# pierluigiferrari/ssd_keras

Hardware: AMD Instinct MI355X
Metric: images/sec SSD300 fwd+decode @batch32 (higher is better)
Workload: dtype f32 (decode, threshold, TF-style f32 NMS, top-k); bf16 conv backbone; 1 GPU; SSD300 VGG-16 inference (mode='inference': forward + DecodeDetections), 21 classes, batch 32 per GPU, conf 0.01 / NMS 0.45 / top-200, random-init weights, synthetic 300x300x3 uint8-range images; per_gpu_batch=32, global_batch=32, conv_dtype=bf16, parallelism=replicas x1, launch=hip_graph (forward + DecodeDetections captured once, replayed per step), decode_stream=same stream; DecodeDetections reads the head outputs directly (no y_pred in HBM)

## Files before the change

### ssd_keras_amd/csrc/ssdhip_convh.hip

```cpp
#include <hip/hip_runtime.h>
#include <stdint.h>
#include <stdlib.h>

#include <type_traits>

#include "ssdhip.h"
#include "ssdhip_math.h"

namespace ssdhip {

#ifdef SSDHIP_PROFILE
__device__ unsigned long long g_profh[16];
#define CH_PROF_DECL long long _pt = clock64(); long long _pa[4] = {0, 0, 0, 0}; int _pn = 0;
#define CH_PROF_MARK(i) { const long long _t = clock64(); _pa[i] += _t - _pt; _pt = _t; }
#define CH_PROF_TILE ++_pn;
#define CH_PROF_FLUSH(base) if ((threadIdx.x & 63) == 0) { for (int _i = 0; _i < 4; ++_i) atomicAdd(&g_profh[(base) + _i], (unsigned long long)_pa[_i]); atomicAdd(&g_profh[(base) + 4], (unsigned long long)_pn); }
#else
#define CH_PROF_DECL
#define CH_PROF_MARK(i)
#define CH_PROF_TILE
#define CH_PROF_FLUSH(base)
#endif

typedef unsigned short bf16_t;
// ... 41 lines not shown
__device__ __forceinline__ u32 ch_pkmax_i16(u32 a, u32 b) {
    return __builtin_bit_cast(u32, __builtin_elementwise_max(__builtin_bit_cast(ch_s16x2, a), __builtin_bit_cast(ch_s16x2, b)));
}

__device__ __forceinline__ void ch_bload(u32 voff, i32x4 rsrc, u32 lds_dst, u32 soff) {
    u32 keep;
    lds_dst = (u32)__builtin_amdgcn_readfirstlane((int)lds_dst);
    soff = (u32)__builtin_amdgcn_readfirstlane((int)soff);
    asm volatile("s_mov_b32 %0, m0\n\ts_mov_b32 m0, %3\n\ts_nop 0\n\tbuffer_load_dwordx4 %1, %2, %4 offen lds\n\ts_mov_b32 m0, %0"
                 : "=&s"(keep) : "v"(voff), "s"(rsrc), "s"(lds_dst), "s"(soff) : "memory");
}
__device__ __forceinline__ i32x4 ch_rsrc(const void* base, int num_records) {
    const unsigned long long a = (unsigned long long)(uintptr_t)base;
    i32x4 r;
    r.x = (int)(u32)a;
    r.y = (int)((u32)(a >> 32) & 0xffffu);
    r.z = num_records;
    r.w = 0x00020000;
    return r;
}
__device__ __forceinline__ u32 ch_keep2(u32 m) {
    const ch_s16x2 h = __builtin_bit_cast(ch_s16x2, m);
    const ch_s16x2 a = h & (short)0x7fff;
    const ch_s16x2 k = (h > (short)0) | (a > (short)0x7f80);
    return __builtin_bit_cast(u32, k);
}
typedef _Float16 ch_f16x8 __attribute__((ext_vector_type(8)));
__device__ __forceinline__ u32 ch_split2(float a, float b, u32& lo_out) {
    const _Float16 ha = (_Float16)a, hb = (_Float16)b;
    const _Float16 la = (_Float16)(a - (float)ha), lb = (_Float16)(b - (float)hb);
    lo_out = (u32)__builtin_bit_cast(unsigned short, la) | ((u32)__builtin_bit_cast(unsigned short, lb) << 16);
    return (u32)__builtin_bit_cast(unsigned short, ha) | ((u32)__builtin_bit_cast(unsigned short, hb) << 16);
}

template <int NW, int SPW, int MODE, int CSH, bool POOL, bool SMALL, bool X3 = false, int NWV = 8, bool STK = false, bool MSK = false,
          bool KEEP = false>
__device__ __forceinline__ void convh_body(const ConvHParams& p, unsigned char* lds, const int first_id) {
    constexpr bool G2 = CSH != 0;
    static_assert(!KEEP || (POOL && !X3 && NWV == 8 && !(MODE & (16384 | 1024))), "KEEP: the staged pooled bf16 epilogue, plain waits");
    static_assert(!MSK || (!POOL && !X3 && NWV == 8 && !(MODE & 16384)), "masked outputs: the staged bf16 epilogue without pooling");
    static_assert(!STK || (POOL && !((MODE & 16384) != 0 && !X3)), "stacked-batch tiles: the staged pooled epilogues");
    static_assert(NWV == 8 || (NWV == 4 && !X3), "8 waves, or 4 (bf16 forms only)");
    constexpr int NPI = 16 / NWV;
    constexpr int WPK = 8 / NWV;
    constexpr int TC = G2 ? (1 << CSH) : 1, TR = G2 ? (CH_BN >> CSH) : 1, SC2 = TC + 2;
    static_assert(!POOL || G2, "the pooled epilogue needs 2-D tiles");
    static_assert(!G2 || (TR + 2) * (TC + 2) <= 64 * SPW, "the 2-D slab must fit the slab buffer");
    constexpr bool LZ = (MODE & 8192) != 0 && NW == 4;
    constexpr int D = LZ ? NW - 1 : NW;
    constexpr int SLAB0 = NW * CH_WST, SLB = SPW * 8192;
    constexpr unsigned OOB = 0x80000000u;
    constexpr bool PERSIST = (MODE & 128) != 0;
    static_assert(SPW + D <= 10, "slice cs+1's slab must have landed two steps before tap 8 of slice cs reads it");
    static_assert(SLB >= 32768, "the epilogue stages half a tile (8 waves x 32 positions x 128 B) in the idle slab buffer");

    auto tile_of = [&](const int id, int& q0, int& co0) {
        const int xcd = id & 7, slot = id >> 3;
        const int qt = (slot / p.n_tiles) * 8 + xcd;
        q0 = G2 ? qt : qt * CH_BN;
        co0 = (slot % p.n_tiles) * CH_BM;
        return id < p.total_ids && qt < p.q_tiles;
    };
    int id = first_id, q0, co0;
    if (!tile_of(id, q0, co0)) {
        if constexpr (MSK) {
            if (p.bsum) {
                const int w_ = (int)threadIdx.x >> 6, l_ = (int)threadIdx.x & 63;
                const int slot_ = first_id >> 3, cz = (slot_ % p.n_tiles) * CH_BM + (w_ >> 2) * 64 + l_;
                p.bsum[(size_t)(4 * ((slot_ / p.n_tiles) * 8 + (first_id & 7)) + (w_ & 3)) * p.Cout + cz] = 0.f;
            }
        }
        return;
    }

    const int tid = threadIdx.x, lane = tid & 63;
// ... 68 lines not shown
        }
        int q = tile_q0 - (W + 2) + row0;
        int b = 0, h = 0, w = 0;
        if (q >= 0) { b = q / (H1 * W1); const int r = q - b * (H1 * W1); h = r / W1; w = r - h * W1; }
        else { w = q; }
#pragma unroll
        for (int k = 0; k < NXO; ++k) {
            const int row = row0 + XSTEP * k;
            const int j = (lane & 7) ^ ((row >> 1) & 7);
            const bool ok = w >= 0 && w < W && h < H && q < p.Q && row < SP;
            xoff[k] = ok ? (u32)(((b * H + h) * W + w) * (XC * 2) + j * 16) : OOB;
            q += XSTEP;
            w += XSTEP;
            while (w >= W1) { w -= W1; if (++h == H1) { h = 0; ++b; } }
        }
    };
    make_xoff(q0);
    auto xdst = [&](const int k) { return (u32)((XSTEP * k + 8 * wave) * 128); };
    constexpr int NWP = 2 * WPK;
    u32 woff[NWP];
#pragma unroll
    for (int i = 0; i < NWP; ++i) {
        const int row = (i * NWV + wave) * 8 + (lane >> 3);
        const int j = (lane & 7) ^ ((row >> 1) & 7);
        woff[i] = (u32)(row * (9 * Cin * 2) + j * 16);
    }

    auto issue_w_piece = [&](const int co, const int cs, const int tap, const int stage, const int i) {
        const u32 soff = (u32)(((co * 9 + tap) * Cin + cs * 64) * 2);
        ch_bload(woff[i], rw, lds0 + stage * CH_WST + (i * NWV + wave) * 1024, soff);
    };

    u32 abase[4];
    {
        const int row = wm * 64 + r31;
#pragma unroll
        for (int kk = 0; kk < 4; ++kk) abase[kk] = (u32)(row * 128 + (((2 * kk + khalf) ^ ((row >> 1) & 7)) << 4));
    }
    const int slot2 = wn * (16 * NPI) + r31;
    const int prow = G2 ? (2 * (slot2 >> CSH)) * SC2 + (slot2 & (TC - 1)) : wn * (32 * NPI) + r31;
    auto pirow = [&](const int pi) {
        return G2 ? (pi >> 1) * (2 * (32 >> CSH)) * SC2 + (pi & 1) * SC2 : pi * 32;
    };

    f32x16 acc[2][NPI];
    bf16x8 fa[2][4][2], fb[2][4][NPI];

    u32 ra[4], rb[NPI], re[NPI];
    auto read_addr = [&](const int cs, const int tap, const int stage) {
        u32 wst = (u32)(stage * CH_WST);
        u32 toff = (u32)((tap / 3) * (G2 ? SC2 : W1) + tap % 3);
        u32 sl = (u32)(SLAB0 + (cs & 1) * SLB);
        asm volatile("" : "+s"(wst), "+s"(toff), "+s"(sl));
#pragma unroll
        for (int kk = 0; kk < 4; ++kk) ra[kk] = abase[kk] + wst;
#pragma unroll
        for (int pi = 0; pi < NPI; ++pi) {
            const u32 row = (u32)(prow + pirow(pi)) + toff;
            rb[pi] = sl + (row << 7);
            re[pi] = (((row >> 1) & 7u) ^ (u32)khalf) << 4;
        }
    };
    constexpr int RPK = 2 + NPI;
    auto read_one = [&](auto setc, auto jc) {
        constexpr int S = decltype(setc)::value, j = decltype(jc)::value, kk = j / RPK, w = j % RPK;
        if constexpr (w < 2) fa[S][kk][w] = *reinterpret_cast<const bf16x8*>(lds + ra[kk] + w * 4096);
        else fb[S][kk][w - 2] = *reinterpret_cast<const bf16x8*>(lds + rb[w - 2] + (re[w - 2] ^ (u32)(kk << 5)));
    };
    auto mfma_one = [&](auto setc, auto ic) {
        constexpr int S = decltype(setc)::value, i = decltype(ic)::value, kk = i / (2 * NPI), ci = (i / NPI) & 1, pi = i % NPI;
        if constexpr (X3)
            acc[ci][pi] = __builtin_amdgcn_mfma_f32_32x32x16_f16(__builtin_bit_cast(ch_f16x8, fa[S][kk][ci]), __builtin_bit_cast(ch_f16x8, fb[S][kk][pi]),
                                                                 acc[ci][pi], 0, 0, 0);
        else
            acc[ci][pi] = __builtin_amdgcn_mfma_f32_32x32x16_bf16(fa[S][kk][ci], fb[S][kk][pi], acc[ci][pi], 0, 0, 0);
    };
    using I0 = std::integral_constant<int, 0>; using I1 = std::integral_constant<int, 1>;

#pragma unroll
    for (int k = 0; k < NXO; ++k) ch_bload(xoff[k], rx, lds0 + SLAB0 + xdst(k), 0u);
#pragma unroll
    for (int d = 0; d < D; ++d)
#pragma unroll
        for (int i = 0; i < NWP; ++i) issue_w_piece(co0, 0, d, d, i);
    asm volatile("s_waitcnt vmcnt(%0)" :: "n"(NWP * (D - 2)) : "memory");
    __builtin_amdgcn_s_barrier();
    read_addr(0, 0, 0);
#pragma unroll
    for (int kk = 0; kk < 4; ++kk) {
#pragma unroll
        for (int ci = 0; ci < 2; ++ci) fa[0][kk][ci] = *reinterpret_cast<const bf16x8*>(lds + ra[kk] + ci * 4096);
#pragma unroll
        for (int pi = 0; pi < NPI; ++pi) fb[0][kk][pi] = *reinterpret_cast<const bf16x8*>(lds + rb[pi] + (re[pi] ^ (u32)(kk << 5)));
    }

    int vbase = 0;
    bool has_next = false;
    int q0n = 0, co0n = 0;

    auto step = [&](auto grpc, auto setc, auto tapc, const int cs, const bool nomore, const bool nxt) {
        constexpr int GRP = decltype(grpc)::value, S = decltype(setc)::value, TAP = decltype(tapc)::value;
        using Sn = std::integral_constant<int, 1 - S>;
        constexpr auto issued = [](int t, bool lst) { return (lst ? (t < 9 - D ? 2 : 0) : 2 + (t < SPW ? 1 : 0)) * WPK; };
        constexpr int n_mid = (D == 3 ? 0 : (TAP > 0 ? issued(TAP - 1, false) : 2 * WPK)) + issued(TAP, false);
        constexpr int n_last = (D == 3 ? 0 : (TAP > 0 ? issued(TAP - 1, true) : 2 * WPK)) + issued(TAP, true);
        const int vs = vbase + cs;
        const bool post = cs == 0 && vbase > 0;
        const int st = NW == 3 ? (TAP + D) % 3 : ((vs + TAP + D) & 3);
        constexpr int RSH = ((MODE & 64) && GRP) ? 2 : 0, QSH = ((MODE & 8) && GRP) ? 2 : 0;
        auto addr_now = [&]() { read_addr(cs + (TAP == 8 ? 1 : 0), (TAP + 1) % 9, NW == 3 ? (TAP + 1) % 3 : ((vs + TAP + 1) & 3)); };
        auto req_w = [&](const int wi) {
            constexpr bool CARRY = TAP + D >= 9;
            if (!nomore || !CARRY) {
                const bool over = CARRY && nxt;
                issue_w_piece(over ? co0n : co0, over ? 0 : cs + (CARRY ? 1 : 0), (TAP + D) % 9, st, wi);
            }
        };
        auto req_x = [&](const int u) {
            if (!nomore)
                ch_bload(xoff[TAP * WPK + u], rx, lds0 + SLAB0 + ((cs + 1) & 1) * SLB + xdst(TAP * WPK + u),
                         nxt ? 0u : (u32)(((X3 && cs + 1 >= p.nx) ? cs + 1 - p.nx : cs + 1) * 128));
        };
        auto slot = [&](auto ic) {
            constexpr int i = decltype(ic)::value, j = i - RSH;
            __builtin_amdgcn_sched_barrier(0);
            if constexpr (!(MODE & 32)) mfma_one(setc, ic);
            __builtin_amdgcn_sched_barrier(0);
            if constexpr (i == 0) {
                addr_now();
                __builtin_amdgcn_sched_barrier(0);
            }
            if constexpr (NWV == 8) {
                if constexpr (!(MODE & 2)) {
                    if constexpr (j >= 0 && j < 4) {
                        read_one(Sn{}, std::integral_constant<int, 2 * (j < 0 ? 0 : j)>{});
                        read_one(Sn{}, std::integral_constant<int, 2 * (j < 0 ? 0 : j) + 1>{});
                    } else if constexpr (j >= 4 && j < 12) {
                        read_one(Sn{}, std::integral_constant<int, (j < 4 ? 4 : j) + 4>{});
                    }
                }
                if constexpr (!(MODE & 1)) {
                    if constexpr (i == 1 + QSH) req_w(0);
                    else if constexpr (i == 5 + QSH) req_w(1);
                    else if constexpr (i == 9 + QSH && TAP < SPW) req_x(0);
                }
            } else {
                if constexpr (!(MODE & 2) && i < 24) read_one(Sn{}, std::integral_constant<int, (i < 24 ? i : 0)>{});
                if constexpr (!(MODE & 1)) {
                    if constexpr (i == 2) req_w(0);
                    else if constexpr (i == 6) req_w(1);
                    else if constexpr (i == 10) req_w(2);
                    else if constexpr (i == 14) req_w(3);
                    else if constexpr ((i == 18 || i == 22) && TAP < SPW) req_x(i == 18 ? 0 : 1);
                }
            }
        };
        slot(std::integral_constant<int, 0>{}); slot(std::integral_constant<int, 1>{}); slot(std::integral_constant<int, 2>{});
        slot(std::integral_constant<int, 3>{}); slot(std::integral_constant<int, 4>{}); slot(std::integral_constant<int, 5>{});
        slot(std::integral_constant<int, 6>{}); slot(std::integral_constant<int, 7>{}); slot(std::integral_constant<int, 8>{});
        slot(std::integral_constant<int, 9>{}); slot(std::integral_constant<int, 10>{}); slot(std::integral_constant<int, 11>{});
        slot(std::integral_constant<int, 12>{}); slot(std::integral_constant<int, 13>{}); slot(std::integral_constant<int, 14>{});
        slot(std::integral_constant<int, 15>{});
        if constexpr (NWV == 4) {
            slot(std::integral_constant<int, 16>{}); slot(std::integral_constant<int, 17>{}); slot(std::integral_constant<int, 18>{});
            slot(std::integral_constant<int, 19>{}); slot(std::integral_constant<int, 20>{}); slot(std::integral_constant<int, 21>{});
            slot(std::integral_constant<int, 22>{}); slot(std::integral_constant<int, 23>{}); slot(std::integral_constant<int, 24>{});
            slot(std::integral_constant<int, 25>{}); slot(std::integral_constant<int, 26>{}); slot(std::integral_constant<int, 27>{});
            slot(std::integral_constant<int, 28>{}); slot(std::integral_constant<int, 29>{}); slot(std::integral_constant<int, 30>{});
            slot(std::integral_constant<int, 31>{});
        }
        __builtin_amdgcn_sched_barrier(0);
        if constexpr (!(MODE & 4)) {
            constexpr bool TOL = (MODE & 1024) != 0 && TAP < D - 2;
            if constexpr (LZ) {
                if (TOL && post) asm volatile("s_waitcnt vmcnt(%0)" :: "n"((MODE & 1) ? 0 : n_mid + NST + 1) : "memory");
                else if (!nomore) asm volatile("s_waitcnt vmcnt(%0)" :: "n"((MODE & 1) ? 0 : n_mid) : "memory");
                else asm volatile("s_waitcnt vmcnt(%0)" :: "n"((MODE & 1) ? 0 : n_last) : "memory");
            } else {
            if (TOL && post) asm volatile("s_waitcnt vmcnt(%0) lgkmcnt(0)" :: "n"((MODE & 1) ? 0 : n_mid + NST + 1) : "memory");
            else if (!nomore) asm volatile("s_waitcnt vmcnt(%0) lgkmcnt(0)" :: "n"((MODE & 1) ? 0 : n_mid) : "memory");
            else asm volatile("s_waitcnt vmcnt(%0) lgkmcnt(0)" :: "n"((MODE & 1) ? 0 : n_last) : "memory");
            }
            __builtin_amdgcn_s_barrier();
        }
    };
    auto slice = [&](auto grpc, auto parc, const int cs, const bool nomore, const bool nxt) {
        constexpr int P = decltype(parc)::value;
        using A = std::integral_constant<int, P>; using B = std::integral_constant<int, 1 - P>;
        step(grpc, A{}, std::integral_constant<int, 0>{}, cs, nomore, nxt); step(grpc, B{}, std::integral_constant<int, 1>{}, cs, nomore, nxt);
        step(grpc, A{}, std::integral_constant<int, 2>{}, cs, nomore, nxt); step(grpc, B{}, std::integral_constant<int, 3>{}, cs, nomore, nxt);
        step(grpc, A{}, std::integral_constant<int, 4>{}, cs, nomore, nxt); step(grpc, B{}, std::integral_constant<int, 5>{}, cs, nomore, nxt);
        step(grpc, A{}, std::integral_constant<int, 6>{}, cs, nomore, nxt); step(grpc, B{}, std::integral_constant<int, 7>{}, cs, nomore, nxt);
        step(grpc, A{}, std::integral_constant<int, 8>{}, cs, nomore, nxt);
    };
    auto k_loop = [&](auto grpc) {
        for (int cs = 0; cs < csteps; cs += 2) {
            const bool fin = cs + 2 >= csteps;
            slice(grpc, I0{}, cs, false, false);
            if (PERSIST && fin && has_next) make_xoff(q0n);
            slice(grpc, I1{}, cs + 1, fin && !has_next, fin && has_next);
        }
    };

    CH_PROF_DECL
    for (;;) {
        if constexpr (PERSIST) has_next = tile_of(id + (int)gridDim.x, q0n, co0n);
        u32 bias_dw;
        {
            const bf16_t* bsrc = (p.bias ? p.bias + co0 + wm * 64 : p.w) + 2 * r31;
            asm volatile("global_load_dword %0, %1, off" : "=v"(bias_dw) : "v"(bsrc) : "memory");
        }
#pragma unroll
        for (int ci = 0; ci < 2; ++ci)
#pragma unroll
            for (int pi = 0; pi < NPI; ++pi)
#pragma unroll
                for (int v = 0; v < 16; ++v) acc[ci][pi][v] = 0.f;
        if constexpr ((MODE & (8 | 64)) != 0) {
            if (wave < 4) k_loop(I0{}); else k_loop(I1{});
        } else {
            k_loop(I0{});
        }

        asm volatile("" : "+v"(bias_dw));
        CH_PROF_MARK(0)
        if constexpr ((MODE & 512) != 0) {
            asm volatile("" :: "v"(acc[0][0]), "v"(acc[0][1]), "v"(acc[1][0]), "v"(acc[1][1]));
            if constexpr (NPI == 4) asm volatile("" :: "v"(acc[0][2]), "v"(acc[0][3]), "v"(acc[1][2]), "v"(acc[1][3]));
        } else {
        unsigned char* stage = lds + SLAB0 + SLB + wave * 4096;
        float bv[2][16];
        if (!p.bias) bias_dw = 0u;
        const float rfloor = p.relu ? 0.f : -__builtin_inff();
        if constexpr (X3) {
#pragma unroll
            for (int ci = 0; ci < 2; ++ci)
#pragma unroll
                for (int g = 0; g < 4; ++g)
#pragma unroll
                    for (int e = 0; e < 4; ++e)
                        bv[ci][4 * g + e] = p.bias32 ? p.bias32[co0 + wm * 64 + ci * 32 + 8 * g + 4 * khalf + e] : 0.f;
        } else
#pragma unroll
        for (int ci = 0; ci < 2; ++ci)
#pragma unroll
            for (int g = 0; g < 4; ++g) {
                const int dw = ci * 16 + 4 * g + 2 * khalf;
                const u32 lo = (u32)__builtin_amdgcn_ds_bpermute(dw * 4, (int)bias_dw);
                const u32 hi = (u32)__builtin_amdgcn_ds_bpermute(dw * 4 + 4, (int)bias_dw);
                bv[ci][4 * g + 0] = __uint_as_float(lo << 16);
                bv[ci][4 * g + 1] = __uint_as_float(lo & 0xffff0000u);
                bv[ci][4 * g + 2] = __uint_as_float(hi << 16);
                bv[ci][4 * g + 3] = __uint_as_float(hi & 0xffff0000u);
            }
        if constexpr (!X3) {
        const u32 floor16 = p.relu ? 0u : 0x80008000u;
        auto pack4 = [&](const int ci, const int pi, const int g, u32& p0, u32& p1) {
            const float s0 = acc[ci][pi][4 * g + 0] + bv[ci][4 * g + 0], s1 = acc[ci][pi][4 * g + 1] + bv[ci][4 * g + 1];
            const float s2 = acc[ci][pi][4 * g + 2] + bv[ci][4 * g + 2], s3 = acc[ci][pi][4 * g + 3] + bv[ci][4 * g + 3];
            p0 = ch_pkmax_i16(ch_pack2(s0, s1), floor16);
            p1 = ch_pkmax_i16(ch_pack2(s2, s3), floor16);
        };
        auto store_runs = [&](const u32 (&lo)[4], const u32 (&hi)[4], const u32 off) {
#pragma unroll
            for (int pr = 0; pr < 2; ++pr) {
                const auto sl = __builtin_amdgcn_permlane32_swap(lo[2 * pr], lo[2 * pr + 1], false, false);
                const auto sh = __builtin_amdgcn_permlane32_swap(hi[2 * pr], hi[2 * pr + 1], false, false);
                store16_at(make_uint4(sl[0], sh[0], sl[1], sh[1]), off + pr * 32);
            }
        };
        if constexpr (POOL && DIRECT) {
            static_assert(NPI == 2, "eight-wave form");
            int b, h0, w0;
            tile_origin(q0, b, h0, w0);
// ... 223 lines not shown
                            q += 8;
                            w += 8;
                            if (!SMALL || W1 >= 8) {
                                const bool wr = w >= W1;
                                w -= wr ? W1 : 0;
                                h += wr ? 1 : 0;
                                const bool hr = h == H1;
                                h = hr ? 0 : h;
                                b += hr ? 1 : 0;
                            } else {
                                while (w >= W1) { w -= W1; if (++h == H1) { h = 0; ++b; } }
                            }
                        }
                }
            }
            [[maybe_unused]] ch_u32x4 mk[NPI][4];
            [[maybe_unused]] float bs[8] = {0.f, 0.f, 0.f, 0.f, 0.f, 0.f, 0.f, 0.f};
            [[maybe_unused]] float4 bold0 = make_float4(0.f, 0.f, 0.f, 0.f), bold1 = bold0;
            [[maybe_unused]] float* brow = nullptr;
            if constexpr (MSK) {
                const __amdgpu_buffer_rsrc_t rm = __builtin_amdgcn_make_buffer_rsrc(const_cast<bf16_t*>(p.mask), 0, p.y_bytes, 0x00020000);
#pragma unroll
                for (int pi = 0; pi < NPI; ++pi)
#pragma unroll
                    for (int j = 0; j < 4; ++j) mk[pi][j] = __builtin_amdgcn_raw_buffer_load_b128(rm, soff[pi][j], 0, 0);
                if (p.bsum && lane < 8) {
                    const int slot0 = first_id >> 3;
                    brow = p.bsum + (size_t)(4 * ((slot0 / p.n_tiles) * 8 + (first_id & 7)) + wn) * p.Cout + co0 + wm * 64 + lane * 8;
                    if (id != first_id) { bold0 = reinterpret_cast<const float4*>(brow)[0]; bold1 = reinterpret_cast<const float4*>(brow)[1]; }
                }
            }
#pragma unroll
            for (int pi = 0; pi < NPI; ++pi) {
#pragma unroll
                for (int ci = 0; ci < 2; ++ci)
#pragma unroll
                    for (int g = 0; g < 4; ++g) {
                        u32 p0, p1;
                        pack4(ci, pi, g, p0, p1);
                        const int chunk = ci * 4 + g;
                        *reinterpret_cast<uint2*>(stage + r31 * 128 + ((chunk ^ (r31 & 7)) << 4) + khalf * 8) = make_uint2(p0, p1);
                    }
                asm volatile("s_waitcnt lgkmcnt(0)" ::: "memory");
#pragma unroll
                for (int j = 0; j < 4; ++j) {
                    const int px = j * 8 + (lane >> 3);
                    uint4 v = *reinterpret_cast<const uint4*>(stage + px * 128 + ((c ^ (px & 7)) << 4));
                    if constexpr (MSK) {
                        v.x &= ch_keep2(mk[pi][j][0]); v.y &= ch_keep2(mk[pi][j][1]);
                        v.z &= ch_keep2(mk[pi][j][2]); v.w &= ch_keep2(mk[pi][j][3]);
                        bs[0] += __uint_as_float(v.x << 16); bs[1] += __uint_as_float(v.x & 0xffff0000u);
                        bs[2] += __uint_as_float(v.y << 16); bs[3] += __uint_as_float(v.y & 0xffff0000u);
                        bs[4] += __uint_as_float(v.z << 16); bs[5] += __uint_as_float(v.z & 0xffff0000u);
                        bs[6] += __uint_as_float(v.w << 16); bs[7] += __uint_as_float(v.w & 0xffff0000u);
                    }
                    store16_at(v, soff[pi][j]);
                }
                asm volatile("s_waitcnt lgkmcnt(0)" ::: "memory");
            }
            if constexpr (MSK) {
                if (p.bsum) {
#pragma unroll
                    for (int q = 0; q < 8; ++q) {
                        bs[q] += __shfl_xor(bs[q], 8);
                        bs[q] += __shfl_xor(bs[q], 16);
                        bs[q] += __shfl_xor(bs[q], 32);
// ... 120 lines not shown
                        w += 8;
                        if (!SMALL || W1 >= 8) {
                            const bool wr = w >= W1;
                            w -= wr ? W1 : 0;
                            h += wr ? 1 : 0;
                            const bool hr = h == H1;
                            h = hr ? 0 : h;
                            b += hr ? 1 : 0;
                        } else {
                            while (w >= W1) { w -= W1; if (++h == H1) { h = 0; ++b; } }
                        }
                    }
                }
                asm volatile("s_waitcnt lgkmcnt(0)" ::: "memory");
              }
            }
        }
        }
        CH_PROF_MARK(1)
        CH_PROF_TILE
        if (!has_next) break;
        __builtin_amdgcn_s_barrier();
        CH_PROF_MARK(2)
        id += (int)gridDim.x;
        q0 = q0n;
        co0 = co0n;
        vbase += csteps;
    }
    if (wave == 0) { CH_PROF_FLUSH(0) }
    if (wave == 4) { CH_PROF_FLUSH(8) }
}
#endif

template <int NW, int SPW, int MODE, int CSH, bool POOL, bool X3 = false, int NWV = 8, bool STK = false, bool MSK = false, bool KEEP = false>
__global__ __launch_bounds__(64 * NWV) void convh_kernel(ConvHParams p) {
#if defined(__HIP_DEVICE_COMPILE__)
    __shared__ __attribute__((aligned(1024))) unsigned char lds[ch_lds_bytes(NW, SPW)];
    convh_body<NW, SPW, MODE, CSH, POOL, SPW == 5, X3, NWV, STK, MSK, KEEP>(p, lds, (int)blockIdx.x);
#endif
}

constexpr int CH_MAX_GROUP = 8;
struct ConvHGroup {
    ConvHParams p[CH_MAX_GROUP];
    int first_id[CH_MAX_GROUP + 1];
    int n;
};

template <int MODE>
__global__ __launch_bounds__(CH_THREADS) void convh_group_kernel(ConvHGroup g) {
#if defined(__HIP_DEVICE_COMPILE__)
    __shared__ __attribute__((aligned(1024))) unsigned char lds[ch_lds_bytes(4, 6)];
    const int G = (int)gridDim.x, total = g.first_id[g.n];
    for (int round = 0;; ++round) {
        const int id = (round & 1) ? (round + 1) * G - 1 - (int)blockIdx.x : round * G + (int)blockIdx.x;
        if (round * G >= total) break;
        if (id >= total) continue;
        int k = 0;
        while (k + 1 < g.n && id >= g.first_id[k + 1]) ++k;
        convh_body<4, 6, MODE, 0, false, true>(g.p[k], lds, id - g.first_id[k]);
    }
#endif
}

constexpr bool convh_has_stk(int mode, bool x3) { return x3 ? mode == 128 : mode == 1152; }
template <int MODE, bool X3 = false>
static void convh_launch(const ConvHParams& p, int geom, int pool, int n_cu, hipStream_t stream) {
    int grid = p.total_ids;
    if ((MODE & 128) && grid > n_cu) grid = n_cu;
    if constexpr ((MODE & 4096) != 0 && !X3) {
        constexpr int M4 = MODE & ~4096;
        const dim3 g(grid), t(256);
        if (geom == 4) {
            if (pool) hipLaunchKernelGGL((convh_kernel<4, 6, M4, 4, true, false, 4>), g, t, 0, stream, p);
            else hipLaunchKernelGGL((convh_kernel<4, 6, M4, 4, false, false, 4>), g, t, 0, stream, p);
        } else if (geom == 5) {
            if (pool) hipLaunchKernelGGL((convh_kernel<4, 6, M4, 5, true, false, 4>), g, t, 0, stream, p);
            else hipLaunchKernelGGL((convh_kernel<4, 6, M4, 5, false, false, 4>), g, t, 0, stream, p);
        }
        else if (p.W <= 30) hipLaunchKernelGGL((convh_kernel<4, 5, M4, 0, false, false, 4>), g, t, 0, stream, p);
        else if (p.W <= 62) hipLaunchKernelGGL((convh_kernel<4, 6, M4, 0, false, false, 4>), g, t, 0, stream, p);
        else hipLaunchKernelGGL((convh_kernel<3, 7, M4, 0, false, false, 4>), g, t, 0, stream, p);
    } else {
    const dim3 g(grid), t(CH_THREADS);
    if constexpr ((MODE & 2048) != 0) {
        if (p.W <= 30) hipLaunchKernelGGL((convh_kernel<4, 5, MODE, 0, false, X3>), g, t, 0, stream, p);
        else if (p.W <= 62) hipLaunchKernelGGL((convh_kernel<4, 6, MODE, 0, false, X3>), g, t, 0, stream, p);
        else hipLaunchKernelGGL((convh_kernel<3, 7, MODE, 0, false, X3>), g, t, 0, stream, p);
    } else
    if (geom == 4) {
        if constexpr (convh_has_stk(MODE, X3)) {
            if (pool && p.Hp) { hipLaunchKernelGGL((convh_kernel<4, 6, MODE, 4, true, X3, 8, true>), g, t, 0, stream, p); return; }
        }
        if (pool) hipLaunchKernelGGL((convh_kernel<4, 6, MODE, 4, true, X3>), g, t, 0, stream, p);
        else hipLaunchKernelGGL((convh_kernel<4, 6, MODE, 4, false, X3>), g, t, 0, stream, p);
    } else if (geom == 5) {
        if constexpr (convh_has_stk(MODE, X3)) {
            if (pool && p.Hp) { hipLaunchKernelGGL((convh_kernel<4, 6, MODE, 5, true, X3, 8, true>), g, t, 0, stream, p); return; }
        }
        if (pool) hipLaunchKernelGGL((convh_kernel<4, 6, MODE, 5, true, X3>), g, t, 0, stream, p);
        else hipLaunchKernelGGL((convh_kernel<4, 6, MODE, 5, false, X3>), g, t, 0, stream, p);
    }
    else if (p.W <= 30) hipLaunchKernelGGL((convh_kernel<4, 5, MODE, 0, false, X3>), g, t, 0, stream, p);
    else if (p.W <= 62) hipLaunchKernelGGL((convh_kernel<4, 6, MODE, 0, false, X3>), g, t, 0, stream, p);
    else hipLaunchKernelGGL((convh_kernel<3, 7, MODE, 0, false, X3>), g, t, 0, stream, p);
    }
}

static void convh_launch_keep(const ConvHParams& p, int geom, int n_cu, hipStream_t stream) {
    int grid = p.total_ids;
    if (grid > n_cu) grid = n_cu;
    const dim3 g(grid), t(CH_THREADS);
    if (geom == 4) {
        if (p.Hp) hipLaunchKernelGGL((convh_kernel<4, 6, 128, 4, true, false, 8, true, false, true>), g, t, 0, stream, p);
        else hipLaunchKernelGGL((convh_kernel<4, 6, 128, 4, true, false, 8, false, false, true>), g, t, 0, stream, p);
    } else {
        if (p.Hp) hipLaunchKernelGGL((convh_kernel<4, 6, 128, 5, true, false, 8, true, false, true>), g, t, 0, stream, p);
        else hipLaunchKernelGGL((convh_kernel<4, 6, 128, 5, true, false, 8, false, false, true>), g, t, 0, stream, p);
    }
}

static int convh_masked_grid(int total_ids, int n_tiles, int n_cu) {
    int grid = total_ids < n_cu ? total_ids : n_cu;
    return (grid / (8 * n_tiles)) * (8 * n_tiles);
}
static void convh_launch_masked(const ConvHParams& p, int geom, int grid, hipStream_t stream) {
    const dim3 g(grid), t(CH_THREADS);
    if (geom == 4) hipLaunchKernelGGL((convh_kernel<4, 6, 128, 4, false, false, 8, false, true>), g, t, 0, stream, p);
    else if (geom == 5) hipLaunchKernelGGL((convh_kernel<4, 6, 128, 5, false, false, 8, false, true>), g, t, 0, stream, p);
    else if (p.W <= 30) hipLaunchKernelGGL((convh_kernel<4, 5, 128, 0, false, false, 8, false, true>), g, t, 0, stream, p);
    else if (p.W <= 62) hipLaunchKernelGGL((convh_kernel<4, 6, 128, 0, false, false, 8, false, true>), g, t, 0, stream, p);
    else hipLaunchKernelGGL((convh_kernel<3, 7, 128, 0, false, false, 8, false, true>), g, t, 0, stream, p);
}

}

using namespace ssdhip;

static int convh_cu_count() {
    static int cu_count = 0;
    if (cu_count == 0) {
        int dev = 0, n = 0;
        if (hipGetDevice(&dev) != hipSuccess || hipDeviceGetAttribute(&n, hipDeviceAttributeMultiprocessorCount, dev) != hipSuccess || n <= 0) n = 256;
        cu_count = (n / 8) * 8 > 0 ? (n / 8) * 8 : 8;
    }
    return cu_count;
}

static bool convh_pick_2d(ConvHParams& p, int B, int H, int W, int pool, int& geom, bool has_stk) {
    long long best = -1;
    p.Hp = 0; p.nB = B; p.hp_magic = 0;
    for (int csh = 4; csh <= 5; ++csh) {
        const long long wt = (W + (1 << csh) - 1) >> csh, ht = (H + (256 >> csh) - 1) / (256 >> csh);
        if (best < 0 || (long long)B * wt * ht < best) { best = (long long)B * wt * ht; geom = csh; p.WT = (int)wt; p.HT = (int)ht; }
    }
    const char* e = getenv("SSDHIP_CONVH_STACK");
    if (pool && has_stk && !(e && atoi(e) == 0)) {
        const long long hp = H + 1 + ((H + 1) & 1);
        for (int csh = 4; csh <= 5; ++csh) {
            const long long tr = 256 >> csh, wt = (W + (1 << csh) - 1) >> csh, ht = ((long long)B * hp + tr - 1) / tr;
            if (wt * ht < best && (ht + 1) * tr * hp < 0x7fffffffLL && tr + 2 <= hp) {
                best = wt * ht; geom = csh; p.WT = (int)wt; p.HT = (int)ht;
                p.Hp = (int)hp; p.hp_magic = (unsigned)(0x100000000ULL / (unsigned long long)hp) + 1u;
            }
        }
    }
    if (best > 0x3fffff00LL) return false;
    p.Q = 0;
    p.q_tiles = (int)best;
    return true;
}

static bool convh_plan_unpooled(ConvHParams& p, int B, int H, int W, int n_tiles, int& geom) {
    geom = 0;
    p.HT = p.WT = 0;
    p.Hp = 0;
    if (W > 94) return convh_pick_2d(p, B, H, W, 0, geom, false);
    const long long Q = (long long)B * (H + 1) * (W + 1);
    if (Q > 0x3fffff00LL) return false;
// ... 63 lines not shown
        for (int j = i; j > 0 && Cin_h[order[j]] > Cin_h[order[j - 1]]; --j) { const int t = order[j]; order[j] = order[j - 1]; order[j - 1] = t; }
    ConvHGroup g;
    long long ids = 0;
    for (int s = 0; s < n_problems; ++s) {
        const int k = order[s];
        const int B = B_h[k], H = H_h[k], W = W_h[k], Cin = Cin_h[k], Cout = Cout_h[k];
        const void* x = x_h[k]; const void* weight = weight_h[k]; const void* bias = bias_h ? bias_h[k] : nullptr; void* y = y_h[k];
        if (!x || !weight || !y || B <= 0 || H <= 0 || W <= 0 || W > 62) return SSDHIP_E_BADARG;
        if (Cin <= 0 || (Cin % 128) || Cout <= 0 || (Cout % CH_BM)) return SSDHIP_E_BADARG;
        if (((uintptr_t)x | (uintptr_t)weight | (uintptr_t)y) & 15 || ((uintptr_t)bias & 1)) return SSDHIP_E_BADARG;
        const long long xb = (long long)B * H * W * Cin * 2, wb = (long long)Cout * 9 * Cin * 2, Q = (long long)B * (H + 1) * (W + 1);
        if (xb >= 0x7ffff000LL || wb >= 0x7ffff000LL || (long long)B * H * W * Cout * 2 >= 0x7ffff000LL || Q > 0x3fffff00LL) return SSDHIP_E_BADARG;
        ConvHParams& p = g.p[s];
        p.x = static_cast<const bf16_t*>(x); p.w = static_cast<const bf16_t*>(weight); p.bias = static_cast<const bf16_t*>(bias);
        p.y = static_cast<bf16_t*>(y);
        p.H = H; p.W = W; p.Cin = Cin; p.Cout = Cout; p.relu = relu ? 1 : 0;
        p.Ho = (H + 1) / 2; p.Wo = (W + 1) / 2; p.HT = p.WT = 0;
        p.os = 1; p.ooff = 0; p.Hs = H; p.Ws = W;
        p.Q = (int)Q;
        p.q_tiles = (int)((Q + CH_BN - 1) / CH_BN);
        p.n_tiles = Cout / CH_BM;
        p.x_bytes = (int)xb; p.w_bytes = (int)wb; p.y_bytes = (int)((long long)B * H * W * Cout * 2);
        p.total_ids = ((p.q_tiles + 7) / 8) * p.n_tiles * 8;
        g.first_id[s] = (int)ids;
        ids += p.total_ids;
        if (ids > 0x3fffffffLL) return SSDHIP_E_BADARG;
    }
    for (int s = n_problems; s <= CH_MAX_GROUP; ++s) g.first_id[s] = (int)ids;
    for (int s = n_problems; s < CH_MAX_GROUP; ++s) g.p[s] = g.p[0];
    g.n = n_problems;
    int grid = (int)ids;
    if (grid > convh_cu_count()) grid = convh_cu_count();
    if (max_workgroups >= 8 && grid > (max_workgroups / 8) * 8) grid = (max_workgroups / 8) * 8;
    hipLaunchKernelGGL((convh_group_kernel<0>), dim3(grid), dim3(CH_THREADS), 0, stream, g);
    return hipGetLastError() == hipSuccess ? SSDHIP_OK : SSDHIP_E_LAUNCH;
}

extern "C" int ssdhip_conv3x3_halo_x3_nhwc_f16(const void* x, const void* weight, const float* bias, void* y, int B, int H, int W, int C,
                                               int Cout, int relu, int pool, float oscale, void* stream_) {
    hipStream_t stream = static_cast<hipStream_t>(stream_);
    if (!x || !weight || !y || B <= 0 || H <= 0 || W <= 0 || !(oscale > 0.f)) return SSDHIP_E_BADARG;
    const bool c64 = C == 64;
    if (C <= 0 || ((C % 128) && !c64) || Cout <= 0 || (Cout % CH_BM)) return SSDHIP_E_BADARG;
    if (((uintptr_t)x | (uintptr_t)weight | (uintptr_t)y) & 15 || ((uintptr_t)bias & 3)) return SSDHIP_E_BADARG;
    const int Kc = c64 ? 256 : 3 * C;
    const long long xb = (long long)B * H * W * 2 * C * 2, wb = (long long)Cout * 9 * Kc * 2;
    const int Ho = pool ? (H + 1) / 2 : H, Wo = pool ? (W + 1) / 2 : W;
    const long long yb = (long long)B * Ho * Wo * 2 * Cout * 2;
    if (xb >= 0x7ffff000LL || wb >= 0x7ffff000LL || yb >= 0x7ffff000LL) return SSDHIP_E_BADARG;
    ConvHParams p;
    p.x = static_cast<const bf16_t*>(x); p.w = static_cast<const bf16_t*>(weight); p.bias = nullptr;
    p.y = static_cast<bf16_t*>(y);
    p.H = H; p.W = W; p.Cin = Kc; p.Cout = Cout; p.relu = relu ? 1 : 0;
    p.Ho = (H + 1) / 2; p.Wo = (W + 1) / 2;
    p.HT = p.WT = 0;
    p.os = 1; p.ooff = 0; p.Hs = H; p.Ws = W;
    p.xC = 2 * C; p.nx = c64 ? 2 : C / 64; p.bias32 = bias; p.oscale = oscale;
    int geom = 0;
    if (pool) {
        if (!convh_pick_2d(p, B, H, W, pool, geom, true)) return SSDHIP_E_BADARG;
    } else if (!convh_plan_unpooled(p, B, H, W, Cout / CH_BM, geom)) return SSDHIP_E_BADARG;
    p.n_tiles = Cout / CH_BM;
    p.x_bytes = (int)xb; p.w_bytes = (int)wb; p.y_bytes = (int)yb;
    p.total_ids = ((p.q_tiles + 7) / 8) * p.n_tiles * 8;
    convh_launch<128, true>(p, geom, pool, convh_cu_count(), stream);
    return hipGetLastError() == hipSuccess ? SSDHIP_OK : SSDHIP_E_LAUNCH;
}
// ... 13 lines not shown
    p.Ho = (H + 1) / 2; p.Wo = (W + 1) / 2;
    p.HT = p.WT = 0;
    p.os = 1; p.ooff = 0; p.Hs = H; p.Ws = W;
    int mode = pool ? 1152 : 128;
    if (const char* e = getenv("SSDHIP_CONVH_MODE")) mode = atoi(e);
    int geom = 0;
    if (pool) {
        if (!convh_pick_2d(p, B, H, W, pool, geom, mode == 1152)) return SSDHIP_E_BADARG;
    } else if (!convh_plan_unpooled(p, B, H, W, Cout / CH_BM, geom)) return SSDHIP_E_BADARG;
    p.n_tiles = Cout / CH_BM;
    p.x_bytes = (int)xb; p.w_bytes = (int)wb; p.y_bytes = (int)(pool ? (long long)B * p.Ho * p.Wo * Cout * 2 : (long long)B * H * W * Cout * 2);
    p.total_ids = ((p.q_tiles + 7) / 8) * p.n_tiles * 8;
    const int cu_count = convh_cu_count();
#if defined(SSDHIP_PROFILE)
    if (const char* e = getenv("SSDHIP_CONVH_WAVES")) { if (atoi(e) == 4) mode |= 4096; }
    if (const char* e = getenv("SSDHIP_CONVH_LAZY")) { if (atoi(e) == 1) mode |= 8192; }
#endif
    switch (mode) {
        case 1152: convh_launch<1152>(p, geom, pool, cu_count, stream); break;
#if defined(SSDHIP_PROFILE)
        case 4224: convh_launch<128 | 4096>(p, geom, pool, cu_count, stream); break;
        case 5248: convh_launch<1152 | 4096>(p, geom, pool, cu_count, stream); break;
        case 8320: convh_launch<128 | 8192>(p, geom, pool, cu_count, stream); break;
        case 9344: convh_launch<1152 | 8192>(p, geom, pool, cu_count, stream); break;
        case 12416: convh_launch<128 | 8192 | 4096>(p, geom, pool, cu_count, stream); break;
        case 16512: convh_launch<128 | 16384>(p, geom, pool, cu_count, stream); break;
        case 17536: convh_launch<1152 | 16384>(p, geom, pool, cu_count, stream); break;
        case 129: convh_launch<129>(p, geom, pool, cu_count, stream); break;
        case 130: convh_launch<130>(p, geom, pool, cu_count, stream); break;
        case 135: convh_launch<135>(p, geom, pool, cu_count, stream); break;
        case 384: convh_launch<384>(p, geom, pool, cu_count, stream); break;
        case 640: convh_launch<640>(p, geom, pool, cu_count, stream); break;
#endif
        default: convh_launch<128>(p, geom, pool, cu_count, stream); break;
    }
    return hipGetLastError() == hipSuccess ? SSDHIP_OK : SSDHIP_E_LAUNCH;
}

#ifdef SSDHIP_PROFILE
extern "C" int ssdhip_profile_read_convh(unsigned long long* host_out, int reset) {
    if (hipMemcpyFromSymbol(host_out, HIP_SYMBOL(g_profh), sizeof(g_profh)) != hipSuccess) return -1;
    if (reset) { unsigned long long z[16] = {0}; if (hipMemcpyToSymbol(HIP_SYMBOL(g_profh), z, sizeof(z)) != hipSuccess) return -1; }
    return 0;
}
#endif

static bool convh_masked_plan(ConvHParams& p, int B, int H, int W, int Cout, int& geom) {
    if (!convh_plan_unpooled(p, B, H, W, Cout / CH_BM, geom)) return false;
    p.n_tiles = Cout / CH_BM;
    p.total_ids = ((p.q_tiles + 7) / 8) * p.n_tiles * 8;
    return true;
}

extern "C" int ssdhip_conv3x3_halo_masked_bias_rows(int B, int H, int W, int Cout) {
    if (B <= 0 || H <= 0 || W <= 0 || Cout <= 0 || (Cout % CH_BM)) return 0;
    ConvHParams p;
    int geom;
    if (!convh_masked_plan(p, B, H, W, Cout, geom)) return 0;
    const int grid = convh_masked_grid(p.total_ids, p.n_tiles, convh_cu_count());
    return grid > 0 ? 4 * grid / p.n_tiles : 0;
}

extern "C" int ssdhip_conv3x3_halo_masked_nhwc_bf16(const void* x, const void* weight, const void* mask, void* y, float* bias_partial,
                                                    int bias_rows, int B, int H, int W, int Cin, int Cout, void* stream_) {
    hipStream_t stream = static_cast<hipStream_t>(stream_);
    if (!x || !weight || !mask || !y || B <= 0 || H <= 0 || W <= 0) return SSDHIP_E_BADARG;
    if (Cin <= 0 || (Cin % 128) || Cout <= 0 || (Cout % CH_BM)) return SSDHIP_E_BADARG;
// ... 44 lines not shown
```

Baseline: 16410 images/sec.

## Add 16x16x32 bf16 MFMA path for unpooled 1-D halo conv tiles

Adds an M16 variant of the halo conv body that uses mfma_f32_16x16x32_bf16 instead of 32x32x16. It comes with a new A/B fragment addressing scheme, a permuted position mapping, bias unpacking through ds_bpermute, a reworked prefetch schedule over 32 slots, and a matching staged epilogue. It is enabled by default (env opt-out) for the grouped conv kernel and for unpooled 1-D-tile default-mode launches. The aim is to cut padding waste and improve the MFMA instruction mix for small spatial tiles, at the cost of more LDS reads per FLOP and a more complex schedule.

```diff
diff --git a/ssd_keras_amd/csrc/ssdhip_convh.hip b/ssd_keras_amd/csrc/ssdhip_convh.hip
--- a/ssd_keras_amd/csrc/ssdhip_convh.hip
+++ b/ssd_keras_amd/csrc/ssdhip_convh.hip
@@ -97,15 +97,22 @@
     lo_out = (u32)__builtin_bit_cast(unsigned short, la) | ((u32)__builtin_bit_cast(unsigned short, lb) << 16);
     return (u32)__builtin_bit_cast(unsigned short, ha) | ((u32)__builtin_bit_cast(unsigned short, hb) << 16);
 }
+typedef float f32x4 __attribute__((ext_vector_type(4)));
+__device__ __forceinline__ int ch_m16_pos(const int i) {
+    const int j = (i + 12) & 15;
+    return ((j & 7) << 1) | (j >> 3);
+}
 
 template <int NW, int SPW, int MODE, int CSH, bool POOL, bool SMALL, bool X3 = false, int NWV = 8, bool STK = false, bool MSK = false,
-          bool KEEP = false>
+          bool KEEP = false, bool M16 = false>
 __device__ __forceinline__ void convh_body(const ConvHParams& p, unsigned char* lds, const int first_id) {
     constexpr bool G2 = CSH != 0;
     static_assert(!KEEP || (POOL && !X3 && NWV == 8 && !(MODE & (16384 | 1024))), "KEEP: the staged pooled bf16 epilogue, plain waits");
     static_assert(!MSK || (!POOL && !X3 && NWV == 8 && !(MODE & 16384)), "masked outputs: the staged bf16 epilogue without pooling");
     static_assert(!STK || (POOL && !((MODE & 16384) != 0 && !X3)), "stacked-batch tiles: the staged pooled epilogues");
     static_assert(NWV == 8 || (NWV == 4 && !X3), "8 waves, or 4 (bf16 forms only)");
+    static_assert(!M16 || (CSH == 0 && !POOL && !X3 && NWV == 8 && !MSK && !KEEP && !(MODE & (8 | 64 | 512 | 2048 | 8192 | 16384))),
+                  "16x16x32: the padded position grid with the staged bf16 epilogue");
     constexpr int NPI = 16 / NWV;
     constexpr int WPK = 8 / NWV;
     constexpr int TC = G2 ? (1 << CSH) : 1, TR = G2 ? (CH_BN >> CSH) : 1, SC2 = TC + 2;
@@ -240,48 +247,66 @@
     };
 
     u32 abase[4];
-    {
+    [[maybe_unused]] const int l16 = lane & 15, c4 = lane >> 4;
+    if constexpr (M16) {
+        const int row = wm * 64 + l16;
+#pragma unroll
+        for (int kb = 0; kb < 2; ++kb) abase[kb] = (u32)(row * 128 + (((4 * kb + c4) ^ ((row >> 1) & 7)) << 4));
+    } else {
         const int row = wm * 64 + r31;
 #pragma unroll
         for (int kk = 0; kk < 4; ++kk) abase[kk] = (u32)(row * 128 + (((2 * kk + khalf) ^ ((row >> 1) & 7)) << 4));
     }
     const int slot2 = wn * (16 * NPI) + r31;
-    const int prow = G2 ? (2 * (slot2 >> CSH)) * SC2 + (slot2 & (TC - 1)) : wn * (32 * NPI) + r31;
+    const int prow = M16 ? wn * 64 + ch_m16_pos(l16) : G2 ? (2 * (slot2 >> CSH)) * SC2 + (slot2 & (TC - 1)) : wn * (32 * NPI) + r31;
     auto pirow = [&](const int pi) {
-        return G2 ? (pi >> 1) * (2 * (32 >> CSH)) * SC2 + (pi & 1) * SC2 : pi * 32;
+        return M16 ? pi * 16 : G2 ? (pi >> 1) * (2 * (32 >> CSH)) * SC2 + (pi & 1) * SC2 : pi * 32;
     };
 
-    f32x16 acc[2][NPI];
-    bf16x8 fa[2][4][2], fb[2][4][NPI];
-
-    u32 ra[4], rb[NPI], re[NPI];
+    constexpr int NKB = M16 ? 2 : 4;
+    constexpr int NCI = M16 ? 4 : 2;
+    constexpr int NPB = M16 ? 4 : NPI;
+    using acc_t = std::conditional_t<M16, f32x4, f32x16>;
+    acc_t acc[NCI][NPB];
+    bf16x8 fa[2][NKB][NCI], fb[2][NKB][NPB];
+
+    u32 ra[4], rb[NPB], re[NPB];
     auto read_addr = [&](const int cs, const int tap, const int stage) {
         u32 wst = (u32)(stage * CH_WST);
         u32 toff = (u32)((tap / 3) * (G2 ? SC2 : W1) + tap % 3);
         u32 sl = (u32)(SLAB0 + (cs & 1) * SLB);
         asm volatile("" : "+s"(wst), "+s"(toff), "+s"(sl));
 #pragma unroll
-        for (int kk = 0; kk < 4; ++kk) ra[kk] = abase[kk] + wst;
-#pragma unroll
-        for (int pi = 0; pi < NPI; ++pi) {
+        for (int kk = 0; kk < NKB; ++kk) ra[kk] = abase[kk] + wst;
+#pragma unroll
+        for (int pi = 0; pi < (M16 ? 1 : NPB); ++pi) {
             const u32 row = (u32)(prow + pirow(pi)) + toff;
             rb[pi] = sl + (row << 7);
-            re[pi] = (((row >> 1) & 7u) ^ (u32)khalf) << 4;
+            if constexpr (M16) re[pi] = (((row >> 1) & 7u) ^ (u32)c4) << 4;
+            else re[pi] = (((row >> 1) & 7u) ^ (u32)khalf) << 4;
         }
     };
-    constexpr int RPK = 2 + NPI;
+    constexpr int RPK = NCI + NPB;
     auto read_one = [&](auto setc, auto jc) {
         constexpr int S = decltype(setc)::value, j = decltype(jc)::value, kk = j / RPK, w = j % RPK;
-        if constexpr (w < 2) fa[S][kk][w] = *reinterpret_cast<const bf16x8*>(lds + ra[kk] + w * 4096);
-        else fb[S][kk][w - 2] = *reinterpret_cast<const bf16x8*>(lds + rb[w - 2] + (re[w - 2] ^ (u32)(kk << 5)));
+        constexpr int CIB = M16 ? 2048 : 4096, KSH = M16 ? 6 : 5;
+        if constexpr (w < NCI) fa[S][kk][w] = *reinterpret_cast<const bf16x8*>(lds + ra[kk] + w * CIB);
+        else if constexpr (M16) fb[S][kk][w - NCI] = *reinterpret_cast<const bf16x8*>(lds + rb[0] + (re[0] ^ (u32)(kk << KSH)) + (w - NCI) * 2048);
+        else fb[S][kk][w - NCI] = *reinterpret_cast<const bf16x8*>(lds + rb[w - NCI] + (re[w - NCI] ^ (u32)(kk << KSH)));
     };
     auto mfma_one = [&](auto setc, auto ic) {
-        constexpr int S = decltype(setc)::value, i = decltype(ic)::value, kk = i / (2 * NPI), ci = (i / NPI) & 1, pi = i % NPI;
+        constexpr int S = decltype(setc)::value, i = decltype(ic)::value;
+        if constexpr (M16) {
+            constexpr int kb = i / 16, ci = (i / 4) & 3, pi = i & 3;
+            acc[ci][pi] = __builtin_amdgcn_mfma_f32_16x16x32_bf16(fa[S][kb][ci], fb[S][kb][pi], acc[ci][pi], 0, 0, 0);
+        } else {
+        constexpr int kk = i / (2 * NPI), ci = (i / NPI) & 1, pi = i % NPI;
         if constexpr (X3)
             acc[ci][pi] = __builtin_amdgcn_mfma_f32_32x32x16_f16(__builtin_bit_cast(ch_f16x8, fa[S][kk][ci]), __builtin_bit_cast(ch_f16x8, fb[S][kk][pi]),
                                                                  acc[ci][pi], 0, 0, 0);
         else
             acc[ci][pi] = __builtin_amdgcn_mfma_f32_32x32x16_bf16(fa[S][kk][ci], fb[S][kk][pi], acc[ci][pi], 0, 0, 0);
+        }
     };
     using I0 = std::integral_constant<int, 0>; using I1 = std::integral_constant<int, 1>;
 
@@ -294,6 +319,15 @@
     asm volatile("s_waitcnt vmcnt(%0)" :: "n"(NWP * (D - 2)) : "memory");
     __builtin_amdgcn_s_barrier();
     read_addr(0, 0, 0);
+    if constexpr (M16) {
+#pragma unroll
+        for (int kb = 0; kb < 2; ++kb) {
+#pragma unroll
+            for (int ci = 0; ci < 4; ++ci) fa[0][kb][ci] = *reinterpret_cast<const bf16x8*>(lds + ra[kb] + ci * 2048);
+#pragma unroll
+            for (int pi = 0; pi < 4; ++pi) fb[0][kb][pi] = *reinterpret_cast<const bf16x8*>(lds + rb[0] + (re[0] ^ (u32)(kb << 6)) + pi * 2048);
+        }
+    } else
 #pragma unroll
     for (int kk = 0; kk < 4; ++kk) {
 #pragma unroll
@@ -338,7 +372,14 @@
                 addr_now();
                 __builtin_amdgcn_sched_barrier(0);
             }
-            if constexpr (NWV == 8) {
+            if constexpr (M16) {
+                if constexpr (!(MODE & 2) && i < 24 && i % 3 != 2) read_one(Sn{}, std::integral_constant<int, (i / 3) * 2 + i % 3>{});
+                if constexpr (!(MODE & 1)) {
+                    if constexpr (i == 2) req_w(0);
+                    else if constexpr (i == 11) req_w(1);
+                    else if constexpr (i == 20 && TAP < SPW) req_x(0);
+                }
+            } else if constexpr (NWV == 8) {
                 if constexpr (!(MODE & 2)) {
                     if constexpr (j >= 0 && j < 4) {
                         read_one(Sn{}, std::integral_constant<int, 2 * (j < 0 ? 0 : j)>{});
@@ -369,7 +410,7 @@
         slot(std::integral_constant<int, 9>{}); slot(std::integral_constant<int, 10>{}); slot(std::integral_constant<int, 11>{});
         slot(std::integral_constant<int, 12>{}); slot(std::integral_constant<int, 13>{}); slot(std::integral_constant<int, 14>{});
         slot(std::integral_constant<int, 15>{});
-        if constexpr (NWV == 4) {
+        if constexpr (NWV == 4 || M16) {
             slot(std::integral_constant<int, 16>{}); slot(std::integral_constant<int, 17>{}); slot(std::integral_constant<int, 18>{});
             slot(std::integral_constant<int, 19>{}); slot(std::integral_constant<int, 20>{}); slot(std::integral_constant<int, 21>{});
             slot(std::integral_constant<int, 22>{}); slot(std::integral_constant<int, 23>{}); slot(std::integral_constant<int, 24>{});
@@ -419,11 +460,11 @@
             asm volatile("global_load_dword %0, %1, off" : "=v"(bias_dw) : "v"(bsrc) : "memory");
         }
 #pragma unroll
-        for (int ci = 0; ci < 2; ++ci)
-#pragma unroll
-            for (int pi = 0; pi < NPI; ++pi)
-#pragma unroll
-                for (int v = 0; v < 16; ++v) acc[ci][pi][v] = 0.f;
+        for (int ci = 0; ci < NCI; ++ci)
+#pragma unroll
+            for (int pi = 0; pi < NPB; ++pi)
+#pragma unroll
+                for (int v = 0; v < (M16 ? 4 : 16); ++v) acc[ci][pi][v] = 0.f;
         if constexpr ((MODE & (8 | 64)) != 0) {
             if (wave < 4) k_loop(I0{}); else k_loop(I1{});
         } else {
@@ -437,7 +478,7 @@
             if constexpr (NPI == 4) asm volatile("" :: "v"(acc[0][2]), "v"(acc[0][3]), "v"(acc[1][2]), "v"(acc[1][3]));
         } else {
         unsigned char* stage = lds + SLAB0 + SLB + wave * 4096;
-        float bv[2][16];
+        float bv[NCI][M16 ? 4 : 16];
         if (!p.bias) bias_dw = 0u;
         const float rfloor = p.relu ? 0.f : -__builtin_inff();
         if constexpr (X3) {
@@ -448,6 +489,17 @@
 #pragma unroll
                     for (int e = 0; e < 4; ++e)
                         bv[ci][4 * g + e] = p.bias32 ? p.bias32[co0 + wm * 64 + ci * 32 + 8 * g + 4 * khalf + e] : 0.f;
+        } else if constexpr (M16) {
+#pragma unroll
+            for (int ci = 0; ci < 4; ++ci) {
+                const int dw = ci * 8 + 2 * c4;
+                const u32 lo = (u32)__builtin_amdgcn_ds_bpermute(dw * 4, (int)bias_dw);
+                const u32 hi = (u32)__builtin_amdgcn_ds_bpermute(dw * 4 + 4, (int)bias_dw);
+                bv[ci][0] = __uint_as_float(lo << 16);
+                bv[ci][1] = __uint_as_float(lo & 0xffff0000u);
+                bv[ci][2] = __uint_as_float(hi << 16);
+                bv[ci][3] = __uint_as_float(hi & 0xffff0000u);
+            }
         } else
 #pragma unroll
         for (int ci = 0; ci < 2; ++ci)
@@ -737,6 +789,19 @@
             }
 #pragma unroll
             for (int pi = 0; pi < NPI; ++pi) {
+                if constexpr (M16) {
+#pragma unroll
+                    for (int h = 0; h < 2; ++h) {
+                        const int row = h * 16 + ch_m16_pos(l16);
+#pragma unroll
+                        for (int ci = 0; ci < 4; ++ci) {
+                            u32 p0, p1;
+                            pack4(ci, 2 * pi + h, 0, p0, p1);
+                            const int chunk = 2 * ci + (c4 >> 1);
+                            *reinterpret_cast<uint2*>(stage + row * 128 + ((chunk ^ (row & 7)) << 4) + (c4 & 1) * 8) = make_uint2(p0, p1);
+                        }
+                    }
+                } else
 #pragma unroll
                 for (int ci = 0; ci < 2; ++ci)
 #pragma unroll
@@ -923,11 +988,12 @@
 }
 #endif
 
-template <int NW, int SPW, int MODE, int CSH, bool POOL, bool X3 = false, int NWV = 8, bool STK = false, bool MSK = false, bool KEEP = false>
+template <int NW, int SPW, int MODE, int CSH, bool POOL, bool X3 = false, int NWV = 8, bool STK = false, bool MSK = false, bool KEEP = false,
+          bool M16 = false>
 __global__ __launch_bounds__(64 * NWV) void convh_kernel(ConvHParams p) {
 #if defined(__HIP_DEVICE_COMPILE__)
     __shared__ __attribute__((aligned(1024))) unsigned char lds[ch_lds_bytes(NW, SPW)];
-    convh_body<NW, SPW, MODE, CSH, POOL, SPW == 5, X3, NWV, STK, MSK, KEEP>(p, lds, (int)blockIdx.x);
+    convh_body<NW, SPW, MODE, CSH, POOL, SPW == 5, X3, NWV, STK, MSK, KEEP, M16>(p, lds, (int)blockIdx.x);
 #endif
 }
 
@@ -938,7 +1004,7 @@
     int n;
 };
 
-template <int MODE>
+template <int MODE, bool M16 = false>
 __global__ __launch_bounds__(CH_THREADS) void convh_group_kernel(ConvHGroup g) {
 #if defined(__HIP_DEVICE_COMPILE__)
     __shared__ __attribute__((aligned(1024))) unsigned char lds[ch_lds_bytes(4, 6)];
@@ -949,14 +1015,15 @@
         if (id >= total) continue;
         int k = 0;
         while (k + 1 < g.n && id >= g.first_id[k + 1]) ++k;
-        convh_body<4, 6, MODE, 0, false, true>(g.p[k], lds, id - g.first_id[k]);
+        convh_body<4, 6, MODE, 0, false, true, false, 8, false, false, false, M16>(g.p[k], lds, id - g.first_id[k]);
     }
 #endif
 }
 
 constexpr bool convh_has_stk(int mode, bool x3) { return x3 ? mode == 128 : mode == 1152; }
-template <int MODE, bool X3 = false>
+template <int MODE, bool X3 = false, bool M16 = false>
 static void convh_launch(const ConvHParams& p, int geom, int pool, int n_cu, hipStream_t stream) {
+    static_assert(!M16 || (!X3 && (MODE == 128 || MODE == 1152)), "16x16x32: bf16 product modes");
     int grid = p.total_ids;
     if ((MODE & 128) && grid > n_cu) grid = n_cu;
     if constexpr ((MODE & 4096) != 0 && !X3) {
@@ -992,9 +1059,9 @@
         if (pool) hipLaunchKernelGGL((convh_kernel<4, 6, MODE, 5, true, X3>), g, t, 0, stream, p);
         else hipLaunchKernelGGL((convh_kernel<4, 6, MODE, 5, false, X3>), g, t, 0, stream, p);
     }
-    else if (p.W <= 30) hipLaunchKernelGGL((convh_kernel<4, 5, MODE, 0, false, X3>), g, t, 0, stream, p);
-    else if (p.W <= 62) hipLaunchKernelGGL((convh_kernel<4, 6, MODE, 0, false, X3>), g, t, 0, stream, p);
-    else hipLaunchKernelGGL((convh_kernel<3, 7, MODE, 0, false, X3>), g, t, 0, stream, p);
+    else if (p.W <= 30) hipLaunchKernelGGL((convh_kernel<4, 5, MODE, 0, false, X3, 8, false, false, false, M16>), g, t, 0, stream, p);
+    else if (p.W <= 62) hipLaunchKernelGGL((convh_kernel<4, 6, MODE, 0, false, X3, 8, false, false, false, M16>), g, t, 0, stream, p);
+    else hipLaunchKernelGGL((convh_kernel<3, 7, MODE, 0, false, X3, 8, false, false, false, M16>), g, t, 0, stream, p);
     }
 }
 
@@ -1036,6 +1103,11 @@
         cu_count = (n / 8) * 8 > 0 ? (n / 8) * 8 : 8;
     }
     return cu_count;
+}
+
+static bool convh_mfma16() {
+    const char* e = getenv("SSDHIP_CONVH_MFMA16");
+    return !(e && atoi(e) == 0);
 }
 
 static bool convh_pick_2d(ConvHParams& p, int B, int H, int W, int pool, int& geom, bool has_stk) {
@@ -1165,7 +1237,8 @@
     int grid = (int)ids;
     if (grid > convh_cu_count()) grid = convh_cu_count();
     if (max_workgroups >= 8 && grid > (max_workgroups / 8) * 8) grid = (max_workgroups / 8) * 8;
-    hipLaunchKernelGGL((convh_group_kernel<0>), dim3(grid), dim3(CH_THREADS), 0, stream, g);
+    if (convh_mfma16()) hipLaunchKernelGGL((convh_group_kernel<0, true>), dim3(grid), dim3(CH_THREADS), 0, stream, g);
+    else hipLaunchKernelGGL((convh_group_kernel<0>), dim3(grid), dim3(CH_THREADS), 0, stream, g);
     return hipGetLastError() == hipSuccess ? SSDHIP_OK : SSDHIP_E_LAUNCH;
 }
 
@@ -1245,7 +1318,10 @@
         case 384: convh_launch<384>(p, geom, pool, cu_count, stream); break;
         case 640: convh_launch<640>(p, geom, pool, cu_count, stream); break;
 #endif
-        default: convh_launch<128>(p, geom, pool, cu_count, stream); break;
+        default:
+            if (!pool && convh_mfma16()) convh_launch<128, false, true>(p, geom, pool, cu_count, stream);
+            else convh_launch<128>(p, geom, pool, cu_count, stream);
+            break;
     }
     return hipGetLastError() == hipSuccess ? SSDHIP_OK : SSDHIP_E_LAUNCH;
 }
```

Result: faster. 16650 images/sec (median of 6 runs) (+1.5%).
